# vectorch-ai/ScaleLLM

Hardware: AMD Instinct MI355X
Metric: decode tokens/s (Llama-3-8B-shaped step, bs=256, seq=4k; paged-attention HBM roofline + int4-GEMM TFLOP/s alongside) (higher is better)
Workload: dtype bf16 (int4 weights, fp32 accumulate)

## Files before the change

### scalellm_amd/build_shim.py

```python
from __future__ import annotations

import os
import subprocess
import sys
import sysconfig

HERE = os.path.dirname(os.path.abspath(__file__))
CSRC = os.path.join(HERE, "csrc")
SHIM = os.path.join(CSRC, "shim")
ROOT = os.path.dirname(HERE)
OUT = os.path.join(CSRC, "_slm_shim.so")


def build(force: bool = False) -> str:
    import pybind11
    import torch
    from torch.utils import cpp_extension as ce

    from . import build as slm_build
    slm_build.build()
    srcs = [os.path.join(SHIM, f) for f in ("slm_torch_shim.cpp", "slm_qlinear_hip.cpp", "slm_attn_handler_hip.cpp", "slm_llama_hip.cpp", "slm_sampling_hip.cpp", "slm_rejection_sampler_hip.cpp", "slm_moe_hip.cpp", "slm_mla_hip.cpp", "slm_shim_pybind.cpp")]
    deps = srcs + [os.path.join(SHIM, "slm_torch_shim.h"), os.path.join(SHIM, "slm_qlinear_hip.h"), os.path.join(SHIM, "slm_attn_handler_hip.h"), os.path.join(SHIM, "slm_llama_hip.h"),
                   os.path.join(SHIM, "slm_sampling_hip.h"), os.path.join(SHIM, "slm_rejection_sampler_hip.h"), os.path.join(SHIM, "slm_moe_hip.h"), os.path.join(SHIM, "slm_mla_hip.h"),
                   os.path.join(ROOT, "include", "slm_hip.h")]
    if not force and os.path.exists(OUT) and all(os.path.getmtime(OUT) > os.path.getmtime(d) for d in deps):
        return OUT
    tlib = ce.library_paths()[0]
    rocm = os.environ.get("ROCM_PATH", "/opt/rocm")
    inc = [f"-I{p}" for p in ce.include_paths()] + [f"-I{rocm}/include",
        f"-I{sysconfig.get_paths()['include']}", f"-I{pybind11.get_include()}",
        f"-I{os.path.join(ROOT, 'include')}", f"-I{SHIM}"]
    cmd = ["g++", "-O2", "-std=c++17", "-fPIC", "-shared", "-w", "-D__HIP_PLATFORM_AMD__=1",
           "-DUSE_ROCM=1", f"-D_GLIBCXX_USE_CXX11_ABI={int(torch._C._GLIBCXX_USE_CXX11_ABI)}",
           "-DTORCH_EXTENSION_NAME=_slm_shim", *inc, *srcs, "-o", OUT, f"-L{tlib}", f"-L{CSRC}",
           "-ltorch", "-ltorch_cpu", "-lc10", "-lc10_hip", "-ltorch_hip", "-ltorch_python",
           "-lrccl", "-lslm_hip", f"-Wl,-rpath,{tlib}", "-Wl,-rpath,$ORIGIN"]
    subprocess.check_call(cmd)
    print(f"[scalellm_amd.build_shim] built {OUT}")
    return OUT


if __name__ == "__main__":
    build(force="--force" in sys.argv)
```

### scalellm_amd/cpp_host.py

```python
from __future__ import annotations

import importlib.util
import os

_shim = None


def load_shim():
    global _shim
    if _shim is None:
        from .build_shim import build
        path = build()
        spec = importlib.util.spec_from_file_location("_slm_shim", path)
        mod = importlib.util.module_from_spec(spec)
        spec.loader.exec_module(mod)
        _shim = mod
    return _shim


def cpp_params(params):
    shim = load_shim()
    q = shim.InputParameters()
    q.num_sequences = int(params.q_cu_seq_lens.numel() - 1)
    q.q_cu_seq_lens, q.kv_cu_seq_lens = params.q_cu_seq_lens, params.kv_cu_seq_lens
    q.new_cache_slots, q.block_tables, q.cu_block_lens = params.new_cache_slots, params.block_tables, params.cu_block_lens
    q.q_max_seq_len, q.kv_max_seq_len = int(params.q_max_seq_len), int(params.kv_max_seq_len)
    q.kv_total_len = int(getattr(params, "kv_total_len", 0))
    return q


def cpp_sampling_params(sp):
    shim = load_shim()
    q = shim.SamplingParameters()
    names = ["temperatures", "top_p", "top_k", "do_sample", "seeds"]
    if sp.unique_token_ids is not None:
        names += ["frequency_penalties", "presence_penalties", "repetition_penalties", "unique_token_ids",
                  "unique_token_counts", "unique_token_ids_lens"]
    for name in names:
        t = getattr(sp, name)
        if t is not None:
            setattr(q, name, t)
    q.logprobs, q.max_top_logprobs = bool(sp.logprobs), int(sp.max_top_logprobs)
    return q


def from_decode_step(step, block_size: int, max_tokens: int, fused: bool = True, lanes: int = -1,
                     lanes_chain: bool = True, rank: int = 0, world_size: int = 1, kv_step=None):
    from .decode import hf_state_dict
    shim = load_shim()
    s = step.shape
    qa = step.layers[0]["qkv"].quant_args
    if qa.bits != 4 or qa.desc_act:
        raise ValueError("the C++ host step is built for 4-bit, non-act-order checkpoints")
    m = shim.LlamaForCausalLMHip(hidden=s.hidden, n_heads=s.n_heads, n_kv_heads=s.n_kv_heads, head_dim=s.head_dim,
                                 intermediate=s.intermediate, n_layers=s.n_layers, vocab=s.vocab,
                                 max_position=s.max_position, rope_theta=s.rope_theta, rms_eps=s.rms_eps,
                                 quant_method=qa.quant_method, bits=4, group_size=qa.group_size, desc_act=False,
                                 max_tokens=max_tokens, fused=fused, decode_lanes=lanes, lanes_chain=lanes_chain,
                                 device_index=step.device.index or 0, rank=rank, world_size=world_size)
    m.load_state_dict(hf_state_dict(step))
    m.verify_loaded_weights()
    m.set_kv_caches([(L["kv"].key_cache, L["kv"].value_cache) for L in (kv_step or step).layers], block_size)
    m.set_cos_sin_cache(step.attn.handler.cos_sin)
    m.reserve(max_tokens)
    return m
```

### scalellm_amd/csrc/shim/slm_llama_hip.cpp

```cpp
#include "slm_llama_hip.h"

#include <ATen/hip/HIPEvent.h>
#include <ATen/hip/impl/HIPGuardImplMasqueradingAsCUDA.h>
#include <ATen/hip/impl/HIPStreamMasqueradingAsCUDA.h>
#include <c10/hip/HIPGraphsC10Utils.h>

#include <cmath>

#include "slm_hip.h"
#include "slm_rejection_sampler_hip.h"

namespace slm {
namespace {

using Stream = c10::hip::HIPStreamMasqueradingAsCUDA;

int dt(const torch::Tensor& t) { return t.scalar_type() == torch::kBFloat16 ? SLM_BF16 : SLM_F16; }
void* cur(const torch::Tensor& t) {
  return c10::hip::getCurrentHIPStreamMasqueradingAsCUDA(t.device().index()).stream();
}
void ok(int rc, const char* what) {
  TORCH_CHECK(rc == SLM_OK, what, " failed: ", slm_status_string(rc), " (", rc, ")",
              rc == SLM_ERR_LAUNCH ? slm_last_hip_error() : "");
}
// ... 360 lines not shown
  auto delta = L.o->forward(out);
  llm::kernel::rms_norm_residual(ln.normed, ln.resid, delta, L.post_norm, args_.rms_norm_eps);
  const auto gu = L.gate_up->forward(ln.normed);
  auto act = llm::kernel::silu_with_mul(gu);
  delta = L.down->forward(act);
  const auto& nxt = li + 1 < layers_.size() ? layers_[li + 1].input_norm : final_norm_;
  llm::kernel::rms_norm_residual(ln.normed, ln.resid, delta, nxt, args_.rms_norm_eps);
  (void)n;
}

void LlamaForCausalLMHip::run_two_lanes(Lane& l0, Lane& l1, std::vector<KVCache>& kv) {
  const auto dev = options_.device().index();
  const Stream main = c10::hip::getCurrentHIPStreamMasqueradingAsCUDA(dev);
  if (!side_stream_.has_value()) {
    TORCH_CHECK(!capturing(), "LlamaForCausalLMHip: call reserve() before capturing a two-lane step");
    side_stream_ = c10::hip::getStreamFromPoolMasqueradingAsCUDA(false, dev);
  }
  const Stream side = *side_stream_;
  std::vector<std::unique_ptr<at::cuda::CUDAEvent>> events;
  auto record = [&](const Stream& s) {
    events.push_back(std::make_unique<at::cuda::CUDAEvent>());
    events.back()->record(s);
    return events.back().get();
  };
  record(main)->block(side);
  struct ChipFlag { int& f; explicit ChipFlag(int& x) : f(x) { f = SLM_W4_SHARES_CHIP; } ~ChipFlag() { f = 0; } } chip(chip_flag_);
  Lane* lanes[2] = {&l0, &l1};
  const Stream streams[2] = {main, side};
  const size_t n = layers_.size();
  for (int i = 0; i < 2; ++i) {
    c10::hip::HIPStreamGuardMasqueradingAsCUDA g(streams[i]);
    pre_attn(*lanes[i], 0, kv);
  }
  at::cuda::CUDAEvent* prev = nullptr;
  for (size_t li = 0; li < n; ++li) {
    for (int i = 0; i < 2; ++i) {
      c10::hip::HIPStreamGuardMasqueradingAsCUDA g(streams[i]);
      if (prev != nullptr && opt_.lanes_chain) prev->block(streams[i]);
      attn(*lanes[i], li, kv, 1);
      prev = record(streams[i]);
      attn(*lanes[i], li, kv, 2);
      post_attn(*lanes[i], li);
      if (li + 1 < n) pre_attn(*lanes[i], li + 1, kv);
    }
  }
  record(side)->block(main);
}

torch::Tensor LlamaForCausalLMHip::forward(const torch::Tensor& tokens, const torch::Tensor& positions,
                                           std::vector<KVCache>& kv_caches, const InputParameters& input_params) {
  c10::hip::OptionalHIPGuardMasqueradingAsCUDA guard(options_.device());
  const int64_t T = tokens.size(0);
  TORCH_CHECK(T <= opt_.max_tokens, "n_tokens ", T, " > max_tokens ", opt_.max_tokens);
  TORCH_CHECK(kv_caches.size() == layers_.size(), "one KVCache per layer");
  auto resid = resid_.narrow(0, 0, T);
  auto x = embed_.index_select(0, tokens.to(torch::kLong));
  if (parallel_args_.world_size() > 1) {
    TORCH_CHECK(parallel_args_.process_group() != nullptr, "tensor parallelism needs a ProcessGroup");
    std::vector<torch::Tensor> parts;
    for (int r = 0; r < parallel_args_.world_size(); ++r) parts.push_back(torch::empty_like(x));
    parallel_args_.process_group()->allgather(x.contiguous(), parts);
    x = torch::cat(parts, -1);
  }
  resid.copy_(x);
  InputParameters hinted;
  const InputParameters* prm = &input_params;
  if (input_params.kv_total_len == 0 && !capturing()) {
    const int64_t total = uniform_kv_hint(0, input_params.q_cu_seq_lens.size(0) - 1, input_params.q_max_seq_len,
                                          input_params.kv_max_seq_len, input_params.block_tables.numel(),
                                          kv_caches.empty() ? 0 : kv_caches[0].block_size());
    if (total > 0) { hinted = input_params; hinted.kv_total_len = total; prm = &hinted; }
  }
  auto lanes = make_lanes(T, positions, *prm);
  last_lanes_ = static_cast<int>(lanes.size());
  for (auto& ln : lanes) {
    ln.norm_pending = true;
    ln.pend_x = ln.resid; ln.pend_w = layers_[0].input_norm; ln.pend_splits = 0; ln.pend_residual = false;
  }
// ... 119 lines not shown
```

### scalellm_amd/csrc/shim/slm_llama_hip.h

```cpp
#pragma once
#include <torch/torch.h>

#include <ATen/hip/impl/HIPStreamMasqueradingAsCUDA.h>

#include <memory>
#include <optional>
#include <string>
#include <vector>

#include "slm_attn_handler_hip.h"
#include "slm_qlinear_hip.h"
#include "slm_sampling_hip.h"
#include "slm_torch_shim.h"

namespace slm {

struct LlamaArgs {
  int64_t hidden_size = 4096;
  int64_t n_heads = 32;
  int64_t n_kv_heads = 8;
  int64_t head_dim = 128;
  int64_t intermediate_size = 14336;
  int64_t n_layers = 32;
  int64_t vocab_size = 128256;
  int64_t max_position_embeddings = 8192;
  float rope_theta = 500000.0f;
  float rms_norm_eps = 1e-5f;
};

class LlamaForCausalLMHip {
 public:
  struct Options {
    int64_t max_tokens = 256;
    bool fused = true;
    int64_t decode_lanes = -1;
    bool lanes_chain = true;
  };

  LlamaForCausalLMHip(const LlamaArgs& args, const QuantArgs& quant_args, const ParallelArgs& parallel_args,
                      const torch::TensorOptions& options, const Options& opt,
                      std::shared_ptr<FusedAllReduce> fused_allreduce = nullptr,
                      std::shared_ptr<FusedAllReduce> fused_allreduce_lane1 = nullptr);

  void load_state_dict(const StateDict& state_dict);
  void verify_loaded_weights() const;

  void reserve(int64_t n_tokens);

  torch::Tensor forward(const torch::Tensor& tokens, const torch::Tensor& positions,
                        std::vector<KVCache>& kv_caches, const InputParameters& input_params);
  torch::Tensor logits(const torch::Tensor& hidden_states, const torch::Tensor& selected_idxes);
  torch::Tensor decode_step(const torch::Tensor& tokens, const torch::Tensor& positions,
                            std::vector<KVCache>& kv_caches, const InputParameters& input_params,
                            bool return_logits);
  SampleOutput sample_step(const torch::Tensor& tokens, const torch::Tensor& positions,
                           std::vector<KVCache>& kv_caches, const InputParameters& input_params,
                           const SamplingParameters& sampling);
  SampleOutput verify_step(const torch::Tensor& tokens, const torch::Tensor& positions,
                           std::vector<KVCache>& kv_caches, const InputParameters& input_params,
                           const torch::Tensor& draft_token_ids, const torch::Tensor& draft_probs,
                           const SamplingParameters& sampling, bool mask_out_rejected_tokens = true);
  const torch::Tensor& last_verify_logits() const { return verify_logits_; }
  int last_lanes() const { return last_lanes_; }
  HipAttnHandler& handler() { return *handler_; }
  int64_t n_local_heads() const { return n_heads_; }
  int64_t n_local_kv_heads() const { return n_kv_heads_; }

 private:
  struct Layer {
    std::shared_ptr<ColumnParallelQLinearHipImpl> qkv, gate_up;
    std::shared_ptr<RowParallelQLinearHipImpl> o, down;
    torch::Tensor input_norm, post_norm;
  };
  struct Lane {
    int idx = 0;
    FusedAllReduce* far = nullptr;
    int64_t r0 = 0, r1 = 0;
    torch::Tensor positions, resid, normed, qkv, attn, act, gate_up, o_buf, down_buf, q;
    InputParameters params;
    bool norm_pending = false;
    torch::Tensor pend_x, pend_w;
    int pend_splits = 0, pend_slot = 0;
    bool pend_residual = false;
    int qkv_splits = 0;
  };
  StateDict select_qkv(const StateDict& layer_sd) const;
  bool tp_lanes_ok() const;
  int64_t lane_split(int64_t T, const InputParameters& p) const;
  std::vector<Lane> make_lanes(int64_t T, const torch::Tensor& positions, const InputParameters& p);
  void run_norm(Lane& ln);
  void pre_attn(Lane& ln, size_t li, std::vector<KVCache>& kv);
  void attn(Lane& ln, size_t li, std::vector<KVCache>& kv, int phase = 0);
  void post_attn(Lane& ln, size_t li);
  void plain_layer(Lane& ln, size_t li, std::vector<KVCache>& kv);
  void reduce_add_norm(Lane& ln, int which, torch::Tensor& partial, const torch::Tensor& weight, int splits, int slot);
  void run_two_lanes(Lane& l0, Lane& l1, std::vector<KVCache>& kv);
// ... 31 lines not shown
```

### scalellm_amd/csrc/shim/slm_shim_pybind.cpp

```cpp
#include <ATen/hip/impl/HIPGuardImplMasqueradingAsCUDA.h>
#include <ATen/hip/impl/HIPStreamMasqueradingAsCUDA.h>
#include <torch/extension.h>

#include <algorithm>
#include <thread>

#include "slm_attn_handler_hip.h"
#include "slm_llama_hip.h"
#include "slm_mla_hip.h"
#include "slm_moe_hip.h"
#include "slm_qlinear_hip.h"
#include "slm_rejection_sampler_hip.h"
#include "slm_sampling_hip.h"
#include "slm_torch_shim.h"

namespace py = pybind11;

PYBIND11_MODULE(_slm_shim, m) {
  m.doc() = "libtorch shim over libslm_hip (reference C++ operator signatures)";
  m.def("paged_kv_varlen_mha",
        [](torch::Tensor out, const torch::Tensor& query, const torch::Tensor& key_cache,
           const torch::Tensor& value_cache, const torch::Tensor& q_cu_lens,
           const torch::Tensor& kv_cu_lens, const torch::Tensor& block_table,
           const torch::Tensor& block_cu_lens, const std::optional<torch::Tensor>& alibi_slopes,
// ... 223 lines not shown
      .def("reserve", &slm::HipAttnHandler::reserve)
      .def("get_estimate_workspace_size", &slm::HipAttnHandler::get_estimate_workspace_size)
      .def("set_workspace", &slm::HipAttnHandler::set_workspace);
  m.def("attention_forward",
        [](slm::HipAttnHandler& handler, int64_t n_heads, int64_t n_kv_heads, int64_t head_dim,
           int32_t sliding_window, const torch::Tensor& query, const torch::Tensor& key,
           const torch::Tensor& value, const torch::Tensor& positions, slm::KVCache& kv_cache,
           const slm::InputParameters& params) {
          slm::AttentionImpl attn(n_heads, n_kv_heads, head_dim, &handler, sliding_window);
          return attn.forward(query, key, value, positions, kv_cache, params);
        });
  m.def("handler_pos_emb_and_append",
        [](slm::HipAttnHandler& handler, int64_t n_heads, int64_t n_kv_heads, int64_t head_dim,
           torch::Tensor query, torch::Tensor key, const torch::Tensor& value,
           const torch::Tensor& positions, slm::KVCache& kv_cache, const slm::InputParameters& params) {
          slm::AttentionHandler& h = handler;
          const int64_t T = query.size(0);
          auto q = query.view({T, n_heads, head_dim});
          auto k = key.view({T, n_kv_heads, head_dim});
          auto v = value.view({T, n_kv_heads, head_dim});
          std::tie(q, k) = h.apply_pos_emb(q, k, positions);
          h.append_kv_cache(kv_cache, k, v, params);
        });
  struct PyLlama {
    std::unique_ptr<slm::ProcessGroup> pg;
    std::unique_ptr<slm::LlamaForCausalLMHip> model;
    std::vector<slm::KVCache> kv;
  };
  py::class_<PyLlama>(m, "LlamaForCausalLMHip")
      .def(py::init([make_args](int64_t hidden, int64_t n_heads, int64_t n_kv_heads, int64_t head_dim,
                                int64_t intermediate, int64_t n_layers, int64_t vocab, int64_t max_position,
                                double rope_theta, double rms_eps, const std::string& quant_method, int64_t bits,
                                int64_t group_size, bool desc_act, int64_t max_tokens, bool fused,
                                int64_t decode_lanes, bool lanes_chain, torch::ScalarType dtype, int device_index,
                                int rank, int world_size) {
             slm::LlamaArgs a;
             a.hidden_size = hidden; a.n_heads = n_heads; a.n_kv_heads = n_kv_heads; a.head_dim = head_dim;
             a.intermediate_size = intermediate; a.n_layers = n_layers; a.vocab_size = vocab;
             a.max_position_embeddings = max_position; a.rope_theta = static_cast<float>(rope_theta);
             a.rms_norm_eps = static_cast<float>(rms_eps);
             slm::LlamaForCausalLMHip::Options o;
             o.max_tokens = max_tokens; o.fused = fused; o.decode_lanes = decode_lanes; o.lanes_chain = lanes_chain;
             const bool awq = quant_method == "awq";
             auto p = std::make_unique<PyLlama>();
             const torch::Device dev(torch::kCUDA, device_index);
             if (world_size > 1) p->pg = std::make_unique<slm::LocalShardProcessGroup>(rank, world_size, dev);
             p->model = std::make_unique<slm::LlamaForCausalLMHip>(
                 a, make_args(quant_method, bits, group_size, desc_act, false, awq),
                 slm::ParallelArgs(rank, world_size, p->pg.get()), torch::dtype(dtype).device(dev), o);
             return p;
           }),
           py::arg("hidden"), py::arg("n_heads"), py::arg("n_kv_heads"), py::arg("head_dim"), py::arg("intermediate"),
           py::arg("n_layers"), py::arg("vocab"), py::arg("max_position"), py::arg("rope_theta"), py::arg("rms_eps"),
           py::arg("quant_method"), py::arg("bits"), py::arg("group_size"), py::arg("desc_act"), py::arg("max_tokens"),
           py::arg("fused") = true, py::arg("decode_lanes") = -1, py::arg("lanes_chain") = true,
           py::arg("dtype") = torch::kBFloat16, py::arg("device_index") = 0, py::arg("rank") = 0,
           py::arg("world_size") = 1)
      .def("n_local_heads", [](PyLlama& self) { return self.model->n_local_heads(); })
      .def("n_local_kv_heads", [](PyLlama& self) { return self.model->n_local_kv_heads(); })
      .def("load_state_dict",
           [](PyLlama& self, std::unordered_map<std::string, torch::Tensor> sd) {
             self.model->load_state_dict(slm::StateDict(std::move(sd)));
           })
      .def("verify_loaded_weights", [](PyLlama& self) { self.model->verify_loaded_weights(); })
      .def("set_kv_caches",
           [](PyLlama& self, const std::vector<std::pair<torch::Tensor, torch::Tensor>>& caches, int64_t block_size) {
             self.kv.clear();
             for (const auto& kvp : caches) self.kv.emplace_back(kvp.first, kvp.second, block_size);
           })
      .def("set_cos_sin_cache", [](PyLlama& self, const torch::Tensor& t) { self.model->handler().set_cos_sin_cache(t); })
      .def("reserve", [](PyLlama& self, int64_t n_tokens) { self.model->reserve(n_tokens); })
      .def("decode_step",
           [](PyLlama& self, const torch::Tensor& tokens, const torch::Tensor& positions,
              const slm::InputParameters& params, bool return_logits) {
             return self.model->decode_step(tokens, positions, self.kv, params, return_logits);
           },
           py::arg("tokens"), py::arg("positions"), py::arg("params"), py::arg("return_logits") = false)
      .def("sample_step",
           [](PyLlama& self, const torch::Tensor& tokens, const torch::Tensor& positions,
              const slm::InputParameters& params, const slm::SamplingParameters& sampling) {
             return self.model->sample_step(tokens, positions, self.kv, params, sampling);
           },
           py::arg("tokens"), py::arg("positions"), py::arg("params"), py::arg("sampling"))
      .def("verify_step",
           [](PyLlama& self, const torch::Tensor& tokens, const torch::Tensor& positions,
              const slm::InputParameters& params, const torch::Tensor& draft_token_ids,
              const std::optional<torch::Tensor>& draft_probs, const slm::SamplingParameters& sampling,
              bool mask_out_rejected_tokens) {
             return self.model->verify_step(tokens, positions, self.kv, params, draft_token_ids,
                                            draft_probs ? *draft_probs : torch::Tensor(), sampling,
                                            mask_out_rejected_tokens);
           },
           py::arg("tokens"), py::arg("positions"), py::arg("params"), py::arg("draft_token_ids"),
           py::arg("draft_probs"), py::arg("sampling"), py::arg("mask_out_rejected_tokens") = true)
      .def("last_verify_logits", [](PyLlama& self) { return self.model->last_verify_logits(); })
      .def("forward",
           [](PyLlama& self, const torch::Tensor& tokens, const torch::Tensor& positions,
              const slm::InputParameters& params) { return self.model->forward(tokens, positions, self.kv, params); })
      .def("last_lanes", [](PyLlama& self) { return self.model->last_lanes(); });
  py::class_<slm::W4Linear>(m, "W4Linear")
      .def(py::init<const std::string&, const torch::Tensor&, const torch::Tensor&,
                    const torch::Tensor&, const std::optional<torch::Tensor>&, int64_t, int64_t>(),
           py::arg("quant_method"), py::arg("qweight"), py::arg("qzeros"), py::arg("scales"),
           py::arg("g_idx"), py::arg("group_size"), py::arg("bits") = 4)
      .def("forward", &slm::W4Linear::forward, py::arg("input"), py::arg("bias") = std::nullopt,
           py::arg("out") = std::nullopt)
      .def("dequantize", &slm::W4Linear::dequantize)
      .def("in_features", &slm::W4Linear::in_features)
      .def("out_features", &slm::W4Linear::out_features);
  m.def("process_group_test", [](int n_devices) {
    py::gil_scoped_release nogil;
    int n = n_devices > 0 ? n_devices : static_cast<int>(torch::cuda::device_count());
    std::vector<torch::Device> devs;
    for (int i = 0; i < n; ++i) devs.emplace_back(torch::kCUDA, i);
    std::vector<std::unique_ptr<slm::ProcessGroup>> pgs = slm::ProcessGroup::create_process_groups(devs);
    std::vector<int> ok(n, 0);
    std::vector<std::thread> threads;
    for (int r = 0; r < n; ++r)
      threads.emplace_back([&, r]() {
        c10::hip::HIPGuardMasqueradingAsCUDA guard(devs[r]);
        auto opt = torch::dtype(torch::kHalf).device(devs[r]);
        for (int rep = 0; rep < 3; ++rep) {
          auto t = torch::full({10, 10}, static_cast<float>(r + 1), opt);
          pgs[r]->allreduce(t);
          const bool ar = torch::equal(t.cpu(), torch::full({10, 10}, n * (n + 1) / 2.0f, torch::kHalf));
          auto mine = torch::full({4, 8}, static_cast<float>(r + 1), opt);
          auto flat = torch::zeros({n * 4, 8}, opt);
          pgs[r]->allgather(mine, flat);
          std::vector<torch::Tensor> outs;
          for (int q = 0; q < n; ++q) outs.push_back(torch::zeros({4, 8}, opt));
          pgs[r]->allgather(mine, outs);
          bool ag = true;
// ... 86 lines not shown
```

### scalellm_amd/decode.py

```python
from __future__ import annotations

import contextlib
import dataclasses
import os

from dataclasses import dataclass
from typing import List, Optional

import torch

from . import kernels
from .layers import (Attention, ColumnParallelQLinear, HipAttnHandler, InputParameters, KVCache, uniform_kv_hint,
                     QuantArgs, RowParallelQLinear)
from .model_parallel import ParallelArgs


@dataclass
class LlamaShape:
    hidden: int = 4096
    n_heads: int = 32
    n_kv_heads: int = 8
    head_dim: int = 128
    intermediate: int = 14336
    n_layers: int = 32
# ... 55 lines not shown
    div = 1 if fmt == "awq" else 32 // bits
    if "g_idx" in ck:
        return {"qweight": ck["qweight"][k0 // div:k1 // div].contiguous(), "qzeros": ck["qzeros"],
                "scales": ck["scales"], "g_idx": ck["g_idx"][k0:k1].contiguous()}
    return {"qweight": ck["qweight"][k0 // div:k1 // div].contiguous(),
            "qzeros": ck["qzeros"][k0 // group_size:k1 // group_size].contiguous(),
            "scales": ck["scales"][k0 // group_size:k1 // group_size].contiguous()}


def lane_query(shape: "LlamaShape", n_heads: int, n_kv_heads: int, world_size: int, lanes_min: int,
               n_tokens: int, n_seqs: int, q_max_seq_len: int, kv_max_seq_len: int, tp_lanes_ok: bool = False):
    from ._lib import LaneQuery
    q = LaneQuery()
    q.n_tokens, q.n_seqs, q.q_max_seq_len, q.kv_max_seq_len = int(n_tokens), int(n_seqs), int(q_max_seq_len), \
        int(min(kv_max_seq_len, 2 ** 31 - 1))
    q.world_size, q.tp_lanes_ok, q.lanes_min = int(world_size), int(bool(tp_lanes_ok)), int(lanes_min)
    q.n_heads, q.n_kv_heads, q.head_dim = int(n_heads), int(n_kv_heads), int(shape.head_dim)
    q.layer_weight_bytes = (shape.hidden * (n_heads + 2 * n_kv_heads) * shape.head_dim +
                            n_heads * shape.head_dim * shape.hidden +
                            3 * shape.hidden * shape.intermediate // world_size) // 2
    q.kv_elem_bytes = 2
    return q


def two_lane_split(shape: "LlamaShape", n_heads: int, n_kv_heads: int, world_size: int, lanes_min: int,
                   n_tokens: int, n_seqs: int, q_max_seq_len: int, kv_max_seq_len: int,
                   tp_lanes_ok: bool = False) -> int:
    from . import _lib
    q = lane_query(shape, n_heads, n_kv_heads, world_size, lanes_min, n_tokens, n_seqs, q_max_seq_len,
                   kv_max_seq_len, tp_lanes_ok)
    return int(_lib.lib().slm_decode_lane_split(q))


class LlamaDecodeStep:
    def __init__(self, shape: LlamaShape, max_batch_tokens: int, n_blocks: int, block_size: int,
                 parallel_args: Optional[ParallelArgs] = None, quant_method: str = "awq",
                 group_size: int = 128, dtype=torch.bfloat16, device="cuda", seed: int = 0,
                 kv_fill: str = "none", custom_allreduce=None, keep_checkpoint: bool = False,
                 gptq_sym: bool = False, fuse_silu: bool = True, desc_act: bool = False, bits: int = 4):
        pa = parallel_args or ParallelArgs()
        fuse_silu = fuse_silu and (shape.intermediate // pa.world_size) % 32 == 0
        self.ckpt = [] if keep_checkpoint else None
        if isinstance(custom_allreduce, (list, tuple)):
            self.custom_ars = [a for a in custom_allreduce if a is not None]
        else:
            self.custom_ars = [custom_allreduce] if custom_allreduce is not None else []
        self.custom_ar = self.custom_ars[0] if self.custom_ars else None
        self.shape, self.pa, self.dtype, self.device = shape, pa, dtype, torch.device(device)
        self.defer_splitk = os.environ.get("SLM_DEFER_SPLITK", "1") != "0"
        self.fold_norm = os.environ.get("SLM_FOLD_NORM", "1") != "0"
        _lm = os.environ.get("SLM_DECODE_LANES", "auto")
        self.lanes_min = -1 if _lm == "auto" else int(_lm)
        self.lanes_chain = os.environ.get("SLM_DECODE_LANES_CHAIN", "1") != "0"
        self._side_stream = None
        self._lane_bufs = {}
        self._sample_bufs = None
        self.last_lanes = 1
        self._pinned_lanes = None
        tp = pa.world_size
        assert shape.n_heads % tp == 0 and shape.intermediate % tp == 0 and shape.hidden % tp == 0
        self.n_heads = shape.n_heads // tp
        self.n_kv_heads = max(shape.n_kv_heads // tp, 1)
        self.block_size = block_size
        D, H = shape.head_dim, shape.hidden
        gen = torch.Generator(device=self.device).manual_seed(seed * 1000 + 17)
        desc_act = desc_act and quant_method == "gptq"
        qa = QuantArgs(quant_method=quant_method, bits=bits, group_size=group_size,
                       zero_point=(quant_method == "awq"), desc_act=desc_act)
        inv_freq = 1.0 / (shape.rope_theta ** (torch.arange(0, D, 2, dtype=torch.float32,
                                                              device=self.device) / D))
        cos_sin = HipAttnHandler.build_cos_sin(D, shape.max_position, inv_freq)
        handler = HipAttnHandler(sm_scale=D ** -0.5, rotary_dim=D, cos_sin=cos_sin, interleaved=False)
        self.attn = Attention(self.n_heads, self.n_kv_heads, D, handler)
        qkv_n = (self.n_heads + 2 * self.n_kv_heads) * D
        r, nh, nkv = pa.rank, self.n_heads, self.n_kv_heads
        kv_head0 = (r * shape.n_kv_heads) // tp
        q_full, kv_full, inter = shape.n_heads * D, shape.n_kv_heads * D, shape.intermediate
        self.layers = []
        for _ in range(shape.n_layers):
            L = {}
            L["qkv"] = ColumnParallelQLinear(H, qkv_n * tp, False, qa, False, pa, dtype, self.device)
            L["o"] = RowParallelQLinear(q_full, H, False, qa, True, pa, dtype, self.device)
            L["gate_up"] = ColumnParallelQLinear(H, 2 * inter, False, qa, False, pa, dtype, self.device,
                                                 act_mul="silu" if fuse_silu else None)
            L["down"] = RowParallelQLinear(inter, H, False, qa, True, pa, dtype, self.device)
            full = _rand_int4_linear(gen, H, q_full + 2 * kv_full, group_size, quant_method, dtype, self.device,
# ... 56 lines not shown
                else:
                    flat = t.view(-1)
                    if blk is None:
                        n = min(flat.numel(), 128 * 1024 * 1024)
                        blk = torch.randn(n, device=self.device, dtype=self.dtype, generator=gen)
                    reps = (flat.numel() + blk.numel() - 1) // blk.numel()
                    for r in range(reps):
                        seg = flat[r * blk.numel():(r + 1) * blk.numel()]
                        seg.copy_(blk[:seg.numel()])

    def reserve_workspaces(self, n_tokens: int, max_kv_len: int) -> None:
        s = self.shape

        def need_for(rows: int) -> int:
            need = rows * self.n_heads * 256 * (s.head_dim + 2) * 4
            need = max(need, 64 * rows * max(2 * s.intermediate // self.pa.world_size, s.hidden) * 4)
            return min(need, 4 << 30)
        widest = max(s.hidden, (self.n_heads + 2 * self.n_kv_heads) * s.head_dim)
        h0 = 0
        if self.lanes_min != 0 and self._tp_lanes_ok():
            h0 = two_lane_split(s, self.n_heads, self.n_kv_heads, self.pa.world_size,
                                self.lanes_min if self.lanes_min > 0 else 1, n_tokens, n_tokens, 1, 1 << 30,
                                tp_lanes_ok=True)
        for lane, rows in ((0, n_tokens), (1, (n_tokens + 1) // 2)) if 0 < h0 < n_tokens else ((0, n_tokens),):
            with kernels.workspace_lane(lane):
                kernels.reserve_workspace(need_for(rows), self.device, deferred_nbytes=16 * rows * widest * 4)
        if 0 < h0 < n_tokens and self._side_stream is None:
            self._side_stream = torch.cuda.Stream(device=self.device)

    class _Lane:
        __slots__ = ("idx", "r0", "r1", "T", "positions", "params", "resid", "alt", "normed", "qkv",
                     "attn", "act", "gate_up", "o_buf", "down_buf", "pend", "fold", "stream", "q", "ar")

    def _tp_lanes_ok(self) -> bool:
        if self.pa.world_size == 1:
            return True
        if self.custom_ar is not None:
            return len(self.custom_ars) >= 2
        return bool(getattr(self.pa.process_group, "lane_safe", False))

    def _lane_split(self, T: int, params: InputParameters, ar) -> int:
        if not self._tp_lanes_ok():
            return 0
        lanes_min = self.lanes_min
        if self._pinned_lanes is not None:
            lanes_min = 0 if self._pinned_lanes == 1 else 1
        return two_lane_split(self.shape, self.n_heads, self.n_kv_heads, self.pa.world_size, lanes_min, T,
                              params.q_cu_seq_lens.numel() - 1, params.q_max_seq_len, params.kv_max_seq_len,
                              tp_lanes_ok=True)

    def graph_variants(self, n_tokens: int, n_seqs: int, q_max_seq_len: int):
        lanes = [1]
        if self.lanes_min != 0 and self._tp_lanes_ok() and two_lane_split(
                self.shape, self.n_heads, self.n_kv_heads, self.pa.world_size, 1, n_tokens, n_seqs,
                q_max_seq_len, 1 << 30, tp_lanes_ok=True) > 0:
            lanes.append(2)
        uniform = (False, True) if q_max_seq_len == 1 and n_tokens == n_seqs else (False,)
        return [(ln, u) for ln in lanes for u in uniform]

    def graph_variant_for(self, n_tokens: int, params: InputParameters):
        n_seqs = params.q_cu_seq_lens.numel() - 1
        ar = self.custom_ar if self.pa.world_size > 1 else None
        lanes = 2 if self._lane_split(n_tokens, params, ar) > 0 else 1
        total = uniform_kv_hint(getattr(params, "kv_total_len", 0), n_seqs, params.q_max_seq_len,
                                params.kv_max_seq_len, params.block_tables.numel(), self.block_size)
        uniform = (params.q_max_seq_len == 1 and n_tokens == n_seqs and total == n_seqs * params.kv_max_seq_len)
        return lanes, bool(uniform)

    def probe_lanes(self, n_tokens: int, kv_len: int, n_layers: int = 8, reps: int = 3):
        from . import _lib
        ar = self.custom_ar if self.pa.world_size > 1 else None
        q = lane_query(self.shape, self.n_heads, self.n_kv_heads, self.pa.world_size, 1, n_tokens, n_tokens, 1,
                       kv_len, self._tp_lanes_ok())
        if ar is not None or not self._tp_lanes_ok() or int(_lib.lib().slm_decode_lane_split(q)) <= 0:
            return None
        B = self.block_size
        cache_blocks = self.layers[0]["kv"].key_cache.size(0) // B
        if n_tokens * ((kv_len + B - 1) // B) + 2 > cache_blocks or n_tokens > self.buf["resid"].size(0):
            return None
        tokens, positions, params, _ = make_decode_inputs(n_tokens, kv_len, B, self.device, seed=4321,
                                                          vocab=self.shape.vocab)
        all_layers, k = self.layers, max(1, min(n_layers, len(self.layers)))
        slots = params.new_cache_slots.long()
        saved = [(L["kv"].key_cache[slots].clone(), L["kv"].value_cache[slots].clone()) for L in all_layers[:k]]
        times = {}
        try:
            self.layers = all_layers[:k]
            self.reserve_workspaces(n_tokens, kv_len)
            o_buf, down_buf = self.buf["o"][:n_tokens], self.buf["down"][:n_tokens]
            self.buf["resid"][:n_tokens].normal_()
            import gc
            for lanes in (1, 2):
                with self.graph_variant((lanes, True)):
                    self._run_layers(n_tokens, positions, params, o_buf, down_buf, None)
                    torch.cuda.synchronize(self.device)
                    g = torch.cuda.CUDAGraph()
                    gc.collect()
                    gc_was_on = gc.isenabled()
                    gc.disable()
                    try:
                        with torch.cuda.graph(g):
                            self._run_layers(n_tokens, positions, params, o_buf, down_buf, None)
                    finally:
                        if gc_was_on:
                            gc.enable()
                    g.replay()
                    torch.cuda.synchronize(self.device)
                    ts = []
                    for _ in range(reps):
                        e0, e1 = torch.cuda.Event(enable_timing=True), torch.cuda.Event(enable_timing=True)
                        e0.record()
                        g.replay()
                        e1.record()
                        e1.synchronize()
                        ts.append(e0.elapsed_time(e1) * 1e3)
                    times[lanes] = sorted(ts)[len(ts) // 2]
                    del g
        finally:
            self.layers = all_layers
            for L, (k0, v0) in zip(all_layers[:k], saved):
                L["kv"].key_cache[slots] = k0
                L["kv"].value_cache[slots] = v0
        q.lanes_min = -1
        _lib.check(_lib.lib().slm_decode_lane_policy_record(q, float(times[1]), float(times[2])),
                   "slm_decode_lane_policy_record")
        self.last_probe = dict(n_tokens=n_tokens, kv_len=kv_len, layers=k, one_lane_us=round(times[1], 1),
                               two_lane_us=round(times[2], 1))
        return times[1], times[2]

    @contextlib.contextmanager
    def graph_variant(self, variant):
        prev, self._pinned_lanes = self._pinned_lanes, int(variant[0])
        try:
            yield
        finally:
            self._pinned_lanes = prev

    def _make_lanes(self, T: int, positions, params: InputParameters, o_buf, down_buf, ar, fold):
        b = self.buf
        h0 = self._lane_split(T, params, ar)
        ranges = [(0, T)] if h0 <= 0 or h0 >= T else [(0, h0), (h0, T)]
        lanes = []
        for i, (r0, r1) in enumerate(ranges):
            ln = LlamaDecodeStep._Lane()
            ln.idx, ln.r0, ln.r1, ln.T = i, r0, r1, r1 - r0
            ln.positions = positions[r0:r1]
            if len(ranges) == 1:
                ln.params = params
            else:
                st = self._lane_static(i, r1 - r0)
                torch.sub(params.q_cu_seq_lens[r0:r1 + 1], params.q_cu_seq_lens[r0], out=st["q_cu"])
                torch.sub(params.kv_cu_seq_lens[r0:r1 + 1], params.kv_cu_seq_lens[r0], out=st["kv_cu"])
                ln.params = InputParameters(
                    q_cu_seq_lens=st["q_cu"], kv_cu_seq_lens=st["kv_cu"],
                    new_cache_slots=params.new_cache_slots[r0:r1], block_tables=params.block_tables,
                    cu_block_lens=params.cu_block_lens[r0:r1 + 1], q_max_seq_len=params.q_max_seq_len,
                    kv_max_seq_len=params.kv_max_seq_len,
                    kv_total_len=(r1 - r0) * params.kv_max_seq_len
                    if getattr(params, "kv_total_len", 0) == T * params.kv_max_seq_len else -1)
            ln.resid, ln.normed = b["resid"][r0:r1], b["normed"][r0:r1]
# ... 74 lines not shown
            gu = self._norm_then(ln, L["gate_up"], pend, ln.gate_up)
            kernels.silu_and_mul(ln.act, gu)
        delta = L["down"].forward(ln.act, out=ln.down_buf, reduce=False, defer_splitk=defer)
        nxt = self.layers[li + 1]["in_norm"] if li + 1 < len(self.layers) else self.final_norm
        ln.pend = self._reduce_add_norm(ln, 1, delta, nxt, L["down"].deferred if defer else None)

    def _first_norm(self, ln) -> None:
        ln.pend = (ln.resid, None, None, self.layers[0]["in_norm"])
        if not ln.fold:
            self._run_norm(ln, ln.pend)
            ln.pend = None

    def _run_two_lanes(self, l0, l1) -> None:
        main = torch.cuda.current_stream()
        if self._side_stream is None:
            self._side_stream = torch.cuda.Stream(device=self.device)
        side = self._side_stream
        l0.stream, l1.stream = main, side
        fork = torch.cuda.Event()
        fork.record(main)
        side.wait_event(fork)

        def on(ln):
            st = contextlib.ExitStack()
            st.enter_context(torch.cuda.stream(ln.stream))
            st.enter_context(kernels.workspace_lane(ln.idx))
            st.enter_context(kernels.shared_chip())
            return st
        n = len(self.layers)
        for ln in (l0, l1):
            with on(ln):
                self._first_norm(ln)
                self._pre_attn(ln, 0)
        prev = None
        for li in range(n):
            for ln in (l0, l1):
                with on(ln):
                    if prev is not None and self.lanes_chain:
                        ln.stream.wait_event(prev)
                    self._attn(ln, li, phase=1)
                    prev = torch.cuda.Event()
                    prev.record(ln.stream)
                    self._attn(ln, li, phase=2)
                    self._post_attn(ln, li)
                    if li + 1 < n:
                        self._pre_attn(ln, li + 1)
        with on(l1):
            if l1.pend is not None:
                self._run_norm(l1, l1.pend)
                l1.pend = None
        join = torch.cuda.Event()
        join.record(side)
        main.wait_event(join)

    def _run_layers(self, T: int, positions, params: InputParameters, o_buf, down_buf, ar) -> None:
        fold = self.fold_norm and self.pa.world_size == 1 and T <= 4
        lanes = self._make_lanes(T, positions, params, o_buf, down_buf, ar, fold)
        self.last_lanes = len(lanes)
        if len(lanes) == 2:
            self._run_two_lanes(lanes[0], lanes[1])
        else:
            ln = lanes[0]
            self._first_norm(ln)
            for li in range(len(self.layers)):
                self._pre_attn(ln, li)
                self._attn(ln, li)
                self._post_attn(ln, li)
        for ln in lanes:
            if ln.pend is not None:
                self._run_norm(ln, ln.pend)

    def _trunk(self, tokens: torch.Tensor, positions: torch.Tensor, params: InputParameters):
        s, b, pa = self.shape, self.buf, self.pa
        T = tokens.numel()
        if getattr(params, "kv_total_len", 0) == 0 and not torch.cuda.is_current_stream_capturing():
# ... 201 lines not shown
```

Measured before the change: 10640.

## Add selectable lane-chain dependency modes with probe-based autotuning for two-lane decode

Replaces the fixed every-layer cross-lane event chain in the two-lane decode schedule with a configurable edge set (off, every, follow, stagger, periodic resync). A probe times each candidate on the full layer stack and pins the fastest per token bucket when two lanes beat one lane. The aim is to drop cross-stream waits that serialize attention launches across lanes, so the lanes can overlap more freely. Weaker chaining risks contention between lanes and adds probe time and extra bookkeeping.

```diff
diff --git a/scalellm_amd/build_shim.py b/scalellm_amd/build_shim.py
--- a/scalellm_amd/build_shim.py
+++ b/scalellm_amd/build_shim.py
@@ -20,7 +20,7 @@
     from . import build as slm_build
     slm_build.build()
     srcs = [os.path.join(SHIM, f) for f in ("slm_torch_shim.cpp", "slm_qlinear_hip.cpp", "slm_attn_handler_hip.cpp", "slm_llama_hip.cpp", "slm_sampling_hip.cpp", "slm_rejection_sampler_hip.cpp", "slm_moe_hip.cpp", "slm_mla_hip.cpp", "slm_shim_pybind.cpp")]
-    deps = srcs + [os.path.join(SHIM, "slm_torch_shim.h"), os.path.join(SHIM, "slm_qlinear_hip.h"), os.path.join(SHIM, "slm_attn_handler_hip.h"), os.path.join(SHIM, "slm_llama_hip.h"),
+    deps = srcs + [os.path.join(SHIM, "slm_torch_shim.h"), os.path.join(SHIM, "slm_qlinear_hip.h"), os.path.join(SHIM, "slm_attn_handler_hip.h"), os.path.join(SHIM, "slm_llama_hip.h"), os.path.join(SHIM, "slm_lane_chain.h"),
                    os.path.join(SHIM, "slm_sampling_hip.h"), os.path.join(SHIM, "slm_rejection_sampler_hip.h"), os.path.join(SHIM, "slm_moe_hip.h"), os.path.join(SHIM, "slm_mla_hip.h"),
                    os.path.join(ROOT, "include", "slm_hip.h")]
     if not force and os.path.exists(OUT) and all(os.path.getmtime(OUT) > os.path.getmtime(d) for d in deps):
diff --git a/scalellm_amd/cpp_host.py b/scalellm_amd/cpp_host.py
--- a/scalellm_amd/cpp_host.py
+++ b/scalellm_amd/cpp_host.py
@@ -45,18 +45,21 @@
 
 
 def from_decode_step(step, block_size: int, max_tokens: int, fused: bool = True, lanes: int = -1,
-                     lanes_chain: bool = True, rank: int = 0, world_size: int = 1, kv_step=None):
+                     lanes_chain=None, lanes_chain_resync: int = 0, rank: int = 0, world_size: int = 1, kv_step=None):
     from .decode import hf_state_dict
     shim = load_shim()
     s = step.shape
     qa = step.layers[0]["qkv"].quant_args
     if qa.bits != 4 or qa.desc_act:
         raise ValueError("the C++ host step is built for 4-bit, non-act-order checkpoints")
+    if lanes_chain is None:
+        lanes_chain, lanes_chain_resync = step.chain_mode(max_tokens)
     m = shim.LlamaForCausalLMHip(hidden=s.hidden, n_heads=s.n_heads, n_kv_heads=s.n_kv_heads, head_dim=s.head_dim,
                                  intermediate=s.intermediate, n_layers=s.n_layers, vocab=s.vocab,
                                  max_position=s.max_position, rope_theta=s.rope_theta, rms_eps=s.rms_eps,
                                  quant_method=qa.quant_method, bits=4, group_size=qa.group_size, desc_act=False,
-                                 max_tokens=max_tokens, fused=fused, decode_lanes=lanes, lanes_chain=lanes_chain,
+                                 max_tokens=max_tokens, fused=fused, decode_lanes=lanes, lanes_chain=int(lanes_chain),
+                                 lanes_chain_resync=int(lanes_chain_resync),
                                  device_index=step.device.index or 0, rank=rank, world_size=world_size)
     m.load_state_dict(hf_state_dict(step))
     m.verify_loaded_weights()
diff --git a/scalellm_amd/csrc/shim/slm_lane_chain.h b/scalellm_amd/csrc/shim/slm_lane_chain.h
--- /dev/null
+++ b/scalellm_amd/csrc/shim/slm_lane_chain.h
@@ -0,0 +1,33 @@
+#pragma once
+#include <stdexcept>
+#include <string>
+#include <vector>
+
+namespace slm {
+
+enum LaneChainMode : int { kLaneChainOff = 0, kLaneChainEvery = 1, kLaneChainFollow = 2, kLaneChainStagger = 3 };
+
+struct LaneChainEdge {
+  int waiter_lane, waiter_layer, waited_lane, waited_layer;
+};
+
+inline bool operator==(const LaneChainEdge& a, const LaneChainEdge& b) {
+  return a.waiter_lane == b.waiter_lane && a.waiter_layer == b.waiter_layer && a.waited_lane == b.waited_lane &&
+         a.waited_layer == b.waited_layer;
+}
+
+inline std::vector<LaneChainEdge> lane_chain_edges(int mode, int resync, int n_layers) {
+  if (mode < kLaneChainOff || mode > kLaneChainStagger)
+    throw std::invalid_argument("lane_chain_edges: mode " + std::to_string(mode) + " is not one of 0..3");
+  if (resync < 0) throw std::invalid_argument("lane_chain_edges: resync must be >= 0");
+  std::vector<LaneChainEdge> edges;
+  for (int l = 0; l < n_layers; ++l) {
+    const bool every = mode == kLaneChainEvery ||
+                       (mode >= kLaneChainFollow && resync > 0 && l % resync == 0);
+    if (every && l > 0) edges.push_back({0, l, 1, l - 1});
+    if (every || mode == kLaneChainFollow || (mode == kLaneChainStagger && l == 0)) edges.push_back({1, l, 0, l});
+  }
+  return edges;
+}
+
+}
diff --git a/scalellm_amd/csrc/shim/slm_llama_hip.cpp b/scalellm_amd/csrc/shim/slm_llama_hip.cpp
--- a/scalellm_amd/csrc/shim/slm_llama_hip.cpp
+++ b/scalellm_amd/csrc/shim/slm_llama_hip.cpp
@@ -416,18 +416,29 @@
     c10::hip::HIPStreamGuardMasqueradingAsCUDA g(streams[i]);
     pre_attn(*lanes[i], 0, kv);
   }
-  at::cuda::CUDAEvent* prev = nullptr;
+  const bool tp = parallel_args_.world_size() > 1;
+  const int mode = tp && opt_.lanes_chain != kLaneChainOff ? kLaneChainEvery : opt_.lanes_chain;
+  const auto edges = lane_chain_edges(mode, tp ? 0 : opt_.lanes_chain_resync, static_cast<int>(n));
+  std::vector<at::cuda::CUDAEvent*> done[2] = {std::vector<at::cuda::CUDAEvent*>(n, nullptr),
+                                               std::vector<at::cuda::CUDAEvent*>(n, nullptr)};
+  size_t next_edge = 0;
   for (size_t li = 0; li < n; ++li) {
     for (int i = 0; i < 2; ++i) {
       c10::hip::HIPStreamGuardMasqueradingAsCUDA g(streams[i]);
-      if (prev != nullptr && opt_.lanes_chain) prev->block(streams[i]);
+      for (; next_edge < edges.size() && edges[next_edge].waiter_lane == i &&
+             edges[next_edge].waiter_layer == static_cast<int>(li); ++next_edge) {
+        auto* ev = done[edges[next_edge].waited_lane][edges[next_edge].waited_layer];
+        TORCH_CHECK(ev != nullptr, "lane chain: an edge to an attention launch that is not issued yet");
+        ev->block(streams[i]);
+      }
       attn(*lanes[i], li, kv, 1);
-      prev = record(streams[i]);
+      done[i][li] = record(streams[i]);
       attn(*lanes[i], li, kv, 2);
       post_attn(*lanes[i], li);
       if (li + 1 < n) pre_attn(*lanes[i], li + 1, kv);
     }
   }
+  TORCH_CHECK(next_edge == edges.size(), "lane chain: edges out of issue order");
   record(side)->block(main);
 }
 
diff --git a/scalellm_amd/csrc/shim/slm_llama_hip.h b/scalellm_amd/csrc/shim/slm_llama_hip.h
--- a/scalellm_amd/csrc/shim/slm_llama_hip.h
+++ b/scalellm_amd/csrc/shim/slm_llama_hip.h
@@ -9,6 +9,7 @@
 #include <vector>
 
 #include "slm_attn_handler_hip.h"
+#include "slm_lane_chain.h"
 #include "slm_qlinear_hip.h"
 #include "slm_sampling_hip.h"
 #include "slm_torch_shim.h"
@@ -34,7 +35,8 @@
     int64_t max_tokens = 256;
     bool fused = true;
     int64_t decode_lanes = -1;
-    bool lanes_chain = true;
+    int lanes_chain = 1;
+    int lanes_chain_resync = 0;
   };
 
   LlamaForCausalLMHip(const LlamaArgs& args, const QuantArgs& quant_args, const ParallelArgs& parallel_args,
@@ -62,6 +64,12 @@
                            const SamplingParameters& sampling, bool mask_out_rejected_tokens = true);
   const torch::Tensor& last_verify_logits() const { return verify_logits_; }
   int last_lanes() const { return last_lanes_; }
+  void set_lanes_chain(int mode, int resync = 0) {
+    lane_chain_edges(mode, resync, 0);
+    opt_.lanes_chain = mode; opt_.lanes_chain_resync = resync;
+  }
+  int lanes_chain() const { return opt_.lanes_chain; }
+  int lanes_chain_resync() const { return opt_.lanes_chain_resync; }
   HipAttnHandler& handler() { return *handler_; }
   int64_t n_local_heads() const { return n_heads_; }
   int64_t n_local_kv_heads() const { return n_kv_heads_; }
diff --git a/scalellm_amd/csrc/shim/slm_shim_pybind.cpp b/scalellm_amd/csrc/shim/slm_shim_pybind.cpp
--- a/scalellm_amd/csrc/shim/slm_shim_pybind.cpp
+++ b/scalellm_amd/csrc/shim/slm_shim_pybind.cpp
@@ -279,15 +279,18 @@
                                 int64_t intermediate, int64_t n_layers, int64_t vocab, int64_t max_position,
                                 double rope_theta, double rms_eps, const std::string& quant_method, int64_t bits,
                                 int64_t group_size, bool desc_act, int64_t max_tokens, bool fused,
-                                int64_t decode_lanes, bool lanes_chain, torch::ScalarType dtype, int device_index,
-                                int rank, int world_size) {
+                                int64_t decode_lanes, const py::object& lanes_chain, int lanes_chain_resync,
+                                torch::ScalarType dtype, int device_index, int rank, int world_size) {
              slm::LlamaArgs a;
              a.hidden_size = hidden; a.n_heads = n_heads; a.n_kv_heads = n_kv_heads; a.head_dim = head_dim;
              a.intermediate_size = intermediate; a.n_layers = n_layers; a.vocab_size = vocab;
              a.max_position_embeddings = max_position; a.rope_theta = static_cast<float>(rope_theta);
              a.rms_norm_eps = static_cast<float>(rms_eps);
              slm::LlamaForCausalLMHip::Options o;
-             o.max_tokens = max_tokens; o.fused = fused; o.decode_lanes = decode_lanes; o.lanes_chain = lanes_chain;
+             o.max_tokens = max_tokens; o.fused = fused; o.decode_lanes = decode_lanes;
+             o.lanes_chain = py::isinstance<py::bool_>(lanes_chain) ? int(lanes_chain.cast<bool>()) : lanes_chain.cast<int>();
+             o.lanes_chain_resync = lanes_chain_resync;
+             slm::lane_chain_edges(o.lanes_chain, o.lanes_chain_resync, 0);
              const bool awq = quant_method == "awq";
              auto p = std::make_unique<PyLlama>();
              const torch::Device dev(torch::kCUDA, device_index);
@@ -300,7 +303,7 @@
            py::arg("hidden"), py::arg("n_heads"), py::arg("n_kv_heads"), py::arg("head_dim"), py::arg("intermediate"),
            py::arg("n_layers"), py::arg("vocab"), py::arg("max_position"), py::arg("rope_theta"), py::arg("rms_eps"),
            py::arg("quant_method"), py::arg("bits"), py::arg("group_size"), py::arg("desc_act"), py::arg("max_tokens"),
-           py::arg("fused") = true, py::arg("decode_lanes") = -1, py::arg("lanes_chain") = true,
+           py::arg("fused") = true, py::arg("decode_lanes") = -1, py::arg("lanes_chain") = 1, py::arg("lanes_chain_resync") = 0,
            py::arg("dtype") = torch::kBFloat16, py::arg("device_index") = 0, py::arg("rank") = 0,
            py::arg("world_size") = 1)
       .def("n_local_heads", [](PyLlama& self) { return self.model->n_local_heads(); })
@@ -344,7 +347,19 @@
       .def("forward",
            [](PyLlama& self, const torch::Tensor& tokens, const torch::Tensor& positions,
               const slm::InputParameters& params) { return self.model->forward(tokens, positions, self.kv, params); })
-      .def("last_lanes", [](PyLlama& self) { return self.model->last_lanes(); });
+      .def("last_lanes", [](PyLlama& self) { return self.model->last_lanes(); })
+      .def("set_lanes_chain",
+           [](PyLlama& self, const py::object& mode, int resync) {
+             self.model->set_lanes_chain(py::isinstance<py::bool_>(mode) ? int(mode.cast<bool>()) : mode.cast<int>(), resync);
+           },
+           py::arg("mode"), py::arg("resync") = 0)
+      .def("lanes_chain", [](PyLlama& self) { return std::make_pair(self.model->lanes_chain(), self.model->lanes_chain_resync()); });
+  m.def("lane_chain_edges", [](int mode, int resync, int n_layers) {
+    std::vector<std::tuple<int, int, int, int>> out;
+    for (const auto& e : slm::lane_chain_edges(mode, resync, n_layers))
+      out.emplace_back(e.waiter_lane, e.waiter_layer, e.waited_lane, e.waited_layer);
+    return out;
+  }, py::arg("mode"), py::arg("resync"), py::arg("n_layers"));
   py::class_<slm::W4Linear>(m, "W4Linear")
       .def(py::init<const std::string&, const torch::Tensor&, const torch::Tensor&,
                     const torch::Tensor&, const std::optional<torch::Tensor>&, int64_t, int64_t>(),
diff --git a/scalellm_amd/decode.py b/scalellm_amd/decode.py
--- a/scalellm_amd/decode.py
+++ b/scalellm_amd/decode.py
@@ -111,6 +111,26 @@
     return int(_lib.lib().slm_decode_lane_split(q))
 
 
+LANE_CHAIN_OFF, LANE_CHAIN_EVERY, LANE_CHAIN_FOLLOW, LANE_CHAIN_STAGGER = 0, 1, 2, 3
+LANE_CHAIN_CANDIDATES = ((1, 0), (2, 0), (3, 0), (3, 8))
+
+
+def lane_chain_edges(mode: int, resync: int, n_layers: int):
+    mode, resync = int(mode), int(resync)
+    if not 0 <= mode <= 3:
+        raise ValueError(f"lane_chain_edges: mode {mode} is not one of 0..3")
+    if resync < 0:
+        raise ValueError("lane_chain_edges: resync must be >= 0")
+    edges = []
+    for l in range(n_layers):
+        every = mode == LANE_CHAIN_EVERY or (mode >= LANE_CHAIN_FOLLOW and resync > 0 and l % resync == 0)
+        if every and l > 0:
+            edges.append((0, l, 1, l - 1))
+        if every or mode == LANE_CHAIN_FOLLOW or (mode == LANE_CHAIN_STAGGER and l == 0):
+            edges.append((1, l, 0, l))
+    return edges
+
+
 class LlamaDecodeStep:
     def __init__(self, shape: LlamaShape, max_batch_tokens: int, n_blocks: int, block_size: int,
                  parallel_args: Optional[ParallelArgs] = None, quant_method: str = "awq",
@@ -130,7 +150,13 @@
         self.fold_norm = os.environ.get("SLM_FOLD_NORM", "1") != "0"
         _lm = os.environ.get("SLM_DECODE_LANES", "auto")
         self.lanes_min = -1 if _lm == "auto" else int(_lm)
-        self.lanes_chain = os.environ.get("SLM_DECODE_LANES_CHAIN", "1") != "0"
+        _lc = os.environ.get("SLM_DECODE_LANES_CHAIN", "")
+        self.lanes_chain = int(_lc) if _lc else LANE_CHAIN_EVERY
+        self._chain_forced = bool(_lc)
+        self.lanes_chain_resync = int(os.environ.get("SLM_DECODE_LANES_CHAIN_RESYNC", "0"))
+        self._chain_probed = {}
+        self._pinned_chain = None
+        self.last_chain = (LANE_CHAIN_EVERY, 0)
         self._side_stream = None
         self._lane_bufs = {}
         self._sample_bufs = None
@@ -253,6 +279,30 @@
         __slots__ = ("idx", "r0", "r1", "T", "positions", "params", "resid", "alt", "normed", "qkv",
                      "attn", "act", "gate_up", "o_buf", "down_buf", "pend", "fold", "stream", "q", "ar")
 
+    @property
+    def lanes_chain(self) -> int:
+        return self._lanes_chain
+
+    @lanes_chain.setter
+    def lanes_chain(self, mode) -> None:
+        mode = int(mode)
+        lane_chain_edges(mode, 0, 0)
+        self._lanes_chain, self._chain_forced = mode, True
+
+    def chain_mode(self, n_tokens: int, kv_max_seq_len: Optional[int] = None):
+        if self.pa.world_size > 1:
+            return (LANE_CHAIN_OFF if self._lanes_chain == LANE_CHAIN_OFF else LANE_CHAIN_EVERY), 0
+        if self._pinned_chain is not None:
+            return self._pinned_chain
+        if self._chain_forced:
+            return self._lanes_chain, self.lanes_chain_resync
+        hit = self._chain_probed.get((int(n_tokens) + 31) // 32)
+        if hit is not None:
+            kv_len, mode, resync = hit
+            if kv_max_seq_len is None or (kv_max_seq_len > 0 and max(kv_len, kv_max_seq_len) <= 1.5 * min(kv_len, kv_max_seq_len)):
+                return mode, resync
+        return LANE_CHAIN_EVERY, 0
+
     def _tp_lanes_ok(self) -> bool:
         if self.pa.world_size == 1:
             return True
@@ -303,43 +353,54 @@
                                                           vocab=self.shape.vocab)
         all_layers, k = self.layers, max(1, min(n_layers, len(self.layers)))
         slots = params.new_cache_slots.long()
-        saved = [(L["kv"].key_cache[slots].clone(), L["kv"].value_cache[slots].clone()) for L in all_layers[:k]]
-        times = {}
+        saved = [(L["kv"].key_cache[slots].clone(), L["kv"].value_cache[slots].clone()) for L in all_layers]
+        times, chain_us = {}, {}
+        import gc
+
+        def timed(lanes: int) -> float:
+            with self.graph_variant((lanes, True)):
+                self._run_layers(n_tokens, positions, params, o_buf, down_buf, None)
+                torch.cuda.synchronize(self.device)
+                g = torch.cuda.CUDAGraph()
+                gc.collect()
+                gc_was_on = gc.isenabled()
+                gc.disable()
+                try:
+                    with torch.cuda.graph(g):
+                        self._run_layers(n_tokens, positions, params, o_buf, down_buf, None)
+                finally:
+                    if gc_was_on:
+                        gc.enable()
+                g.replay()
+                torch.cuda.synchronize(self.device)
+                ts = []
+                for _ in range(reps):
+                    e0, e1 = torch.cuda.Event(enable_timing=True), torch.cuda.Event(enable_timing=True)
+                    e0.record()
+                    g.replay()
+                    e1.record()
+                    e1.synchronize()
+                    ts.append(e0.elapsed_time(e1) * 1e3)
+                del g
+            return sorted(ts)[len(ts) // 2]
+
         try:
             self.layers = all_layers[:k]
             self.reserve_workspaces(n_tokens, kv_len)
             o_buf, down_buf = self.buf["o"][:n_tokens], self.buf["down"][:n_tokens]
             self.buf["resid"][:n_tokens].normal_()
-            import gc
+            self._pinned_chain = None if self._chain_forced else (LANE_CHAIN_EVERY, 0)
             for lanes in (1, 2):
-                with self.graph_variant((lanes, True)):
-                    self._run_layers(n_tokens, positions, params, o_buf, down_buf, None)
-                    torch.cuda.synchronize(self.device)
-                    g = torch.cuda.CUDAGraph()
-                    gc.collect()
-                    gc_was_on = gc.isenabled()
-                    gc.disable()
-                    try:
-                        with torch.cuda.graph(g):
-                            self._run_layers(n_tokens, positions, params, o_buf, down_buf, None)
-                    finally:
-                        if gc_was_on:
-                            gc.enable()
-                    g.replay()
-                    torch.cuda.synchronize(self.device)
-                    ts = []
-                    for _ in range(reps):
-                        e0, e1 = torch.cuda.Event(enable_timing=True), torch.cuda.Event(enable_timing=True)
-                        e0.record()
-                        g.replay()
-                        e1.record()
-                        e1.synchronize()
-                        ts.append(e0.elapsed_time(e1) * 1e3)
-                    times[lanes] = sorted(ts)[len(ts) // 2]
-                    del g
+                times[lanes] = timed(lanes)
+            if not self._chain_forced and self.pa.world_size == 1 and times[2] < 0.985 * times[1]:
+                self.layers = all_layers
+                for cand in LANE_CHAIN_CANDIDATES:
+                    self._pinned_chain = cand
+                    chain_us[cand] = timed(2)
         finally:
+            self._pinned_chain = None
             self.layers = all_layers
-            for L, (k0, v0) in zip(all_layers[:k], saved):
+            for L, (k0, v0) in zip(all_layers, saved):
                 L["kv"].key_cache[slots] = k0
                 L["kv"].value_cache[slots] = v0
         q.lanes_min = -1
@@ -347,6 +408,16 @@
                    "slm_decode_lane_policy_record")
         self.last_probe = dict(n_tokens=n_tokens, kv_len=kv_len, layers=k, one_lane_us=round(times[1], 1),
                                two_lane_us=round(times[2], 1))
+        if chain_us:
+            base = chain_us[(LANE_CHAIN_EVERY, 0)]
+            best = min(chain_us, key=chain_us.get)
+            chosen = best if chain_us[best] < 0.985 * base else (LANE_CHAIN_EVERY, 0)
+            self._chain_probed[(n_tokens + 31) // 32] = (kv_len, chosen[0], chosen[1])
+            self.last_probe.update(
+                chain_layers=len(all_layers),
+                chain_us={f"{m}" + (f"+resync{r}" if r else ""): round(t, 1) for (m, r), t in chain_us.items()})
+        mode, resync = self.chain_mode(n_tokens, kv_len)
+        self.last_probe.update(chain_mode=mode, chain_resync=resync)
         return times[1], times[2]
 
     @contextlib.contextmanager
@@ -487,15 +558,20 @@
             with on(ln):
                 self._first_norm(ln)
                 self._pre_attn(ln, 0)
-        prev = None
+        mode, resync = self.chain_mode(l0.T + l1.T, l0.params.kv_max_seq_len)
+        self.last_chain = (mode, resync)
+        waits = {}
+        for wl, wli, dl, dli in lane_chain_edges(mode, resync, n):
+            waits.setdefault((wl, wli), []).append((dl, dli))
+        done = {}
         for li in range(n):
             for ln in (l0, l1):
                 with on(ln):
-                    if prev is not None and self.lanes_chain:
-                        ln.stream.wait_event(prev)
+                    for key in waits.get((ln.idx, li), ()):
+                        ln.stream.wait_event(done[key])
                     self._attn(ln, li, phase=1)
-                    prev = torch.cuda.Event()
-                    prev.record(ln.stream)
+                    done[(ln.idx, li)] = ev = torch.cuda.Event()
+                    ev.record(ln.stream)
                     self._attn(ln, li, phase=2)
                     self._post_attn(ln, li)
                     if li + 1 < n:
```

New measurement: 10650 (median of 6 runs). No clear change (+0.2%).
